# buggyyang/CDC_compression

Hardware: AMD Instinct MI355X
Metric: decoded images/sec at 256x256, 500-step x-param (higher is better)
Workload: dtype f32 (f16x2 split products)

## Files before the change

### cdc_compression_amd/csrc/cdc_internal.h

```cpp
#pragma once
#include <stdio.h>
#include <string.h>
#include <stdlib.h>
#include <hip/hip_runtime.h>
#include <map>
#include <mutex>
#include <utility>
#include <stdint.h>

#include <string>
#include <vector>

#include "conv_args.h"

extern "C" char **environ;

namespace cdc {

typedef void (*conv_kernel_fn)(const ConvArgs);
conv_kernel_fn conv_lookup_a(int MB, int NPW, int lnmode);
conv_kernel_fn conv_lookup_b(int MB, int NPW, int lnmode);
conv_kernel_fn conv_lookup_c(int MB, int NPW, int lnmode);
conv_kernel_fn conv_lookup_split(int MB, int NPW);
conv_kernel_fn conv_lookup_split2(int MB, int NPW, int lnmode, int xu = 1);
conv_kernel_fn conv_lookup_split2h(int MB, int NPW, int lnmode, int xu = 1);
conv_kernel_fn conv_lookup_split2hu(int MB, int NPW);

struct ConvShape {
    int Cin, Cout, KH, KW, stride;
    int C0 = 0;
    int Win = 0;
    int nz = 1, pad_x[4] = {0, 0, 0, 0};
    bool allow_split = false;
    int arith = 0;
    bool per_image_w = false;
    int Ho, Wo;
    int B;
    bool need_all_cout;
    int lnmode;
    int max_ksplit = 1;
};
bool conv_make_plan(const ConvShape &s, ConvPlan *plan);
hipError_t conv_launch(ConvArgs a, const ConvPlan &plan, int B, int nz, hipStream_t st);

struct PfShape {
    int Cin, Cout, C0 = 0, KH, KW, nz = 1, Ho, Wo, B;
    bool need_all_cout = false;
    int stride = 1;
    int uf = 0;
    int cop = 0;
    int tz = 1;
};
struct PfPlan {
    int MB, NPW, WM, WP, ring, tiles_x, tiles_y, groups; size_t lds_bytes; int lin = 0;
    int x16 = 0;
    int pf3_epv = 0, pf3_G = 0, pf3_iters = 0;
};
bool pf_make_plan(const PfShape &s, PfPlan *plan);
hipError_t pf_launch(PfArgs a, const PfPlan &plan, int B, int nz, hipStream_t st);
bool pf3_make_plan(const PfArgs &a, int B, int nz, PfPlan *plan);
hipError_t pf3_launch(PfArgs a, const PfPlan &plan, int B, hipStream_t st);
int device_cus();
struct WsPlan { int W, NPB, stride, waves, tiles, groups; size_t lds_bytes; };
struct WsArgs;
bool ws_make_plan(int Cin, int C0, int Cout, int H, int W, int B, int stride, WsPlan *plan);
hipError_t ws_launch(WsArgs a, const WsPlan &plan, hipStream_t st);
struct Ws1Plan { int NPB, waves, tiles, groups; size_t lds_bytes; };
struct Ws1Args;
bool ws1_make_plan(int Cin, int C0, int Cout, int HW, int B, bool per_image_w, Ws1Plan *plan);
hipError_t ws1_launch(Ws1Args a, const Ws1Plan &plan, hipStream_t st);
bool pw_make_plan(const PfShape &s, PfPlan *plan);
hipError_t pw_launch(PfArgs a, const PfPlan &plan, int B, hipStream_t st);
hipError_t pf_pack_launch(const float *src, long long src_bs, void *dst, long long dst_bs, int C, int H, int W, int B,
                          hipStream_t st);
hipError_t c4_pack_launch(const float *src, long long src_bs, float *dst, int C, long long HW, int B, hipStream_t st);
hipError_t pf_unpack_launch(const void *src, long long src_bs, float *dst, long long dst_bs, int C, int H, int W, int B, hipStream_t st);

inline const char *dev_env(const char *name) {
    static const bool on = [] {
        const char *e = ::getenv("CDC_DEV");
        if (e && atoi(e) != 0) return true;
        static const char *const user_level[] = {"CDC_DEV=", "CDC_ARITH=", "CDC_NO_RANGE_GUARD=", "CDC_GRAPH=", "CDC_DEBUG_PLAN=", "CDC_PROF_OPS=",
                                                 "CDC_BENCH_", "CDC_TEST_OBS=", "CDC_SYNC_EACH_OP=", "CDC_HIP_LIB=", "CDC_NO_COMBINE_FUSE="};
        for (char **v = environ; v && *v; ++v) {
            if (strncmp(*v, "CDC_", 4)) continue;
            bool user = false;
            for (const char *u : user_level) user = user || !strncmp(*v, u, strlen(u));
            if (!user) {
                fprintf(stderr, "cdc_hip: %.*s is set but ignored: development switches need CDC_DEV=1\n", (int)strcspn(*v, "="), *v);
                break;
            }
        }
        return false;
    }();
    return on ? ::getenv(name) : nullptr;
}

inline hipError_t ensure_dynamic_lds(const void *fn, size_t bytes) {
    if (bytes <= 64 * 1024) return hipSuccess;
    static std::mutex mu;
    static std::map<std::pair<int, const void *>, size_t> done;
    int dev = 0;
    (void)hipGetDevice(&dev);
    std::lock_guard<std::mutex> lk(mu);
    size_t &have = done[{dev, fn}];
    if (have >= bytes) return hipSuccess;
    hipError_t e = hipFuncSetAttribute(fn, hipFuncAttributeMaxDynamicSharedMemorySize, (int)bytes);
    if (e == hipSuccess) have = bytes;
// ... 181 lines not shown
```

### cdc_compression_amd/csrc/cdc_planner.hip

```cpp
#include "cdc_state.h"

namespace cdcapi {

constexpr int kKsTarget = 1024;

struct Builder {
    cdc_handle *h;
    int B;
    std::vector<void *> *pool;
    int rc = CDC_OK;
    int planB = 0;
    int pb() const { return planB > 0 ? planB : B; }
    std::vector<Op> *cur = nullptr;

    void emit(Op op) {
        op.id = (int)h->op_ms.size();
        h->op_ms.push_back(0); h->op_n.push_back(0); h->op_flops.push_back(op.flops);
        const bool hoisted = cur == &h->pre_ops;
        char buf[160];
        std::visit([&](const auto &payload) { op_label(payload, buf, sizeof buf, hoisted); }, op.p);
        if (hoisted && !strstr(buf, " HOIST") && strlen(buf) + 7 < sizeof buf) strcat(buf, " HOIST");
        h->op_label.push_back(buf);
        (cur ? cur : &h->ops)->push_back(op);
    }
// ... 275 lines not shown
                if (!tr->valid || tr->C != w.Cout || tr->H != Ho || tr->W != Wo || w.transposed || w.stride != 1 ||
                    o.resid_bs != (long long)w.Cout * Ho * Wo || o.resid_cs != (long long)Ho * Wo) {
                    if (!ensure_f32(o.resid, o.resid_bs)) {
                        if (!rc) rc = fail(h, CDC_ERR_UNSUPPORTED, "planes-only residual of a shape the plane-operand kernels do not read");
                        return true;
                    }
                } else {
                    a.resid = nullptr;
                    a.resid_pf = tr->p; a.rpf_bs = tr->bs(); a.rpf_ps = tr->ps(); a.rpf_ys = Wo + 2; a.rpf_zoff = (Wo + 2) + 1;
                }
            }
        if (planB == 0) pf3_make_plan(a, B, w.nz, &op.plan);
        if (debug_plan())
            fprintf(stderr, "[plan] conv %dx%d %d->%d out %dx%d on conv_pf%s_kernel (epv %d, %d workgroups x %d tiles per group)\n", w.KH, w.KW, w.Cin, w.Cout,
                    Ho, Wo, op.plan.pf3_epv ? "3" : "", op.plan.pf3_epv, op.plan.pf3_G, op.plan.pf3_iters);
        const double px = (double)B * Ho * Wo * w.nz;
        return finish(prof, op, 2.0 * px * w.Cout * w.Cin * w.KH * w.KW, 4.0 * ((double)B * w.Cin * H * W + px * w.Cout), a.out == nullptr);
    }

    bool try_pf_uf(const ConvW &w, const float *s0, long long bs0, int H, int W, float *out, long long out_bs, const ConvOpts &o,
                   bool need_all, int prof) {
        PfShape ps;
        if (!pf_on() || o.uf_c != 3 || o.uf_pad != 3 || !pf_uf_form(w, H, W, need_all, &ps)) return false;
        if (o.pre_mean || o.w_bs || o.wsp_bs || o.max_ksplit > 1 || o.resid || o.res3_w || o.stat_mean) return false;
        PfPlan plan;
        if (!pf_make_plan(ps, &plan)) return false;
        PfConvOp op;
        op.plan = plan; op.nz = 1;
        PfArgs &a = op.a;
        memset(&a, 0, sizeof a);
        a.x0 = s0; a.x0_bs = bs0;
        a.C0 = a.Cin = 32; a.H = H; a.W = W;
        a.w = w.wsh; a.w_zs = w.wsp_zs / 8;
        a.KH = 7; a.KW = 1; a.nz = 1;
        a.nchunk = 2; a.COP = w.COP; a.Cout = w.Cout;
        a.acc_scale = w.wscale_inv;
        out_geometry(a, w, H, W);
        a.out = out; a.out_bs = out_bs;
        if (o.emit_pf && bind_out_pf(a, w, out, out_bs, H, W) && o.no_f32) a.out = nullptr;
        const float *c4 = o.pre_add && cur != &h->pre_ops ? pre_add_c4(o.pre_add, w.Cout, H, W, out_bs) : nullptr;
        epilogue(a, w, o);
        if (c4) { a.pre_add = c4; a.pre_c4 = 1; }
        const double px = (double)B * H * W;
        return finish(prof, op, 2.0 * px * w.Cout * w.Cin * 7, 4.0 * ((double)B * 3 * H * W + px * w.Cout), a.out == nullptr);
    }

    bool try_pw(const ConvW &w, const float *s0, int C0, long long bs0, const float *s1, long long bs1, int H, int W,
                float *out, long long out_bs, const ConvOpts &o, bool need_all, int prof) {
        PfShape ps;
        if (h->arith != 1 || dev_env("CDC_NO_PW") || !pw_form(w, s1 ? C0 : 0, H, W, &ps)) return false;
        if (need_all || o.ln_g || o.stat_mean || o.res3_w || o.pf_only) return false;
        if (o.pre_mean && o.pre_mode != 2) return false;
        if (o.w_bs && !o.wsp_bs) return false;
        PfPlan plan;
        if (!pw_make_plan(ps, &plan)) return false;
        if (plan.lin && (o.shift || o.wsp_bs || (long long)w.Cout * H * W != out_bs)) return false;
        if (debug_plan())
            fprintf(stderr, "[plan] conv1x1 PW Cin=%4d Cout=%4d out=%3dx%-3d %s%s| MB=%d NPW=%d WM=%d WP=%d groups=%d R=%d wgs=%d lds=%zu\n", w.Cin, w.Cout,
                    H, W, o.pre_mean ? "pre2 " : "", o.wsp_bs ? "per-image " : "", plan.MB, plan.NPW, plan.WM, plan.WP, plan.groups, plan.ring,
                    plan.tiles_x * plan.tiles_y * B * plan.groups, plan.lds_bytes);
        PwConvOp op;
        op.plan = plan;
        PfArgs &a = op.a;
        memset(&a, 0, sizeof a);
        a.x0 = s0; a.x0_bs = bs0; a.x1 = s1; a.x1_bs = bs1;
        a.C0 = s1 ? C0 : w.Cin; a.Cin = w.Cin; a.H = H; a.W = W;
        a.pre_mean = o.pre_mean; a.pre_rstd = o.pre_mean ? o.pre_rstd : nullptr;
        a.w = w.wsh; a.w_bs = o.wsp_bs / 8;
        a.KH = 1; a.KW = 1; a.nz = 1;
        a.nchunk = w.Cin / 16; a.COP = w.COP; a.Cout = w.Cout;
        a.acc_scale = w.wscale_inv;
        out_geometry(a, w, H, W);
        a.out = out; a.out_bs = out_bs;
        if (o.emit_pf && !plan.lin && (w.Cout % 32) == 0 && bind_out_pf(a, w, out, out_bs, H, W) && o.no_f32) a.out = nullptr;
        epilogue(a, w, o);
        const double px = (double)B * H * W;
        return finish(prof, op, 2.0 * px * w.Cout * w.Cin, 4.0 * ((double)B * w.Cin * H * W + px * w.Cout), a.out == nullptr);
    }

    bool ws_would_plan(const ConvW &w, int C0, bool two_src, int H, int W, WsPlan *plan) {
        if (h->arith != 1 || !w.wsh || planB > 0 || w.KH != 3 || w.KW != 3 || (w.stride != 1 && w.stride != 2) || w.transposed || w.nz != 1) return false;
        if (w.py() != 1 || w.px() != 1) return false;
        if (w.COP != w.Cout || w.Cin_pad != w.Cin) return false;
        if (w.stride == 2 && ((H & 1) || (W & 1) || two_src)) return false;
        return ws_make_plan(w.Cin, two_src ? C0 : w.Cin, w.Cout, H / w.stride, W / w.stride, pb(), w.stride, plan);
    }
    bool try_ws(const ConvW &w, const float *s0, int C0, long long bs0, const float *s1, long long bs1, int H, int W, float *raw,
                long long raw_bs, int prof, const float *pre_add = nullptr) {
        WsConvOp op;
        if (rc || !ws_would_plan(w, C0, s1 != nullptr, H, W, &op.plan)) return false;
        if (!ensure_f32(s0, bs0) || (s1 && !ensure_f32(s1, bs1))) return false;
        const int Ho = H / w.stride, Wo = W / w.stride;
        if (raw_bs != (long long)w.Cout * Ho * Wo) return false;
        WsArgs &a = op.a;
        memset(&a, 0, sizeof a);
        a.x0 = s0; a.x0_bs = bs0; a.x1 = s1; a.x1_bs = bs1;
        a.C0 = s1 ? C0 : w.Cin; a.Cin = w.Cin; a.H = Ho; a.B = B;
        a.w = w.wsh; a.nchunk = w.Cin / 16; a.COP = w.COP; a.Cout = w.Cout; a.acc_scale = w.wscale_inv;
        a.bias = pre_add ? nullptr : w.bias;
        a.pre_add = pre_add;
        a.out = raw; a.out_bs = raw_bs;
        a.fault = fault_flag();
        if (debug_plan())
            fprintf(stderr, "[plan] conv 3x3 s%d %d->%d out %dx%d on conv_ws_kernel: %d tiles of %d pixels x %d groups, %d waves, %zu bytes of LDS\n", w.stride, w.Cin, w.Cout, Ho, Wo,
                    op.plan.tiles, op.plan.NPB * 32, op.plan.groups, op.plan.waves, op.plan.lds_bytes);
        const double px = (double)B * Ho * Wo;
        return finish(prof, op, 2.0 * px * w.Cout * w.Cin * 9, 4.0 * ((double)B * H * W * w.Cin + px * w.Cout), false);
    }

    bool try_ws1(const ConvW &w, const float *s0, int C0, long long bs0, const float *s1, long long bs1, int H, int W, float *out, long long out_bs,
                 const ConvOpts &o, bool need_all, int prof) {
        PfShape ps;
        if (rc || h->arith != 1 || planB > 0 || !pw_form(w, 0, H, W, &ps)) return false;
        if (need_all || o.ln_g || o.stat_mean || o.res3_w || o.pf_only || (o.pre_add && o.resid) || o.relu || o.resid1 || o.uf_c) return false;
        if (o.pre_mean && o.pre_mode != 2) return false;
        if (o.w_bs && !o.wsp_bs) return false;
        if (w.COP != w.Cout || w.Cin_pad != w.Cin || out_bs != (long long)w.Cout * H * W) return false;
        if (o.resid && (o.resid_cs != (long long)H * W)) return false;
        const long long blocks = (long long)pb() * (H * W / 32);
        const long long max_blocks = dev_env("CDC_WS1_MAX_BLOCKS") ? atoll(dev_env("CDC_WS1_MAX_BLOCKS")) : 128;
        const int max_groups_wide = dev_env("CDC_WS1_MAX_GROUPS") ? atoi(dev_env("CDC_WS1_MAX_GROUPS")) : 0;
        const bool wide_ok = blocks <= max_blocks || (max_groups_wide > 0 && blocks <= 256 && w.Cout / 32 <= max_groups_wide);
        if (!wide_ok && !(o.wsp_bs && W < 32)) return false;
        Ws1ConvOp op;
        op.H = H;
        if (!ws1_make_plan(w.Cin, s1 ? C0 : w.Cin, w.Cout, H * W, pb(), o.wsp_bs != 0, &op.plan)) return false;
        if (!ensure_f32(s0, bs0) || (s1 && !ensure_f32(s1, bs1)) || (o.resid && !ensure_f32(o.resid, o.resid_bs))) return false;
        Ws1Args &a = op.a;
// ... 1087 lines not shown
```

### cdc_compression_amd/csrc/cdc_state.h

```cpp
#pragma once
#include <math.h>
#include <stdarg.h>
#include <stdio.h>
#include <stdlib.h>
#include <string.h>

#include <algorithm>
#include <map>
#include <memory>
#include <string>
#include <variant>
#include <vector>

#include "../../include/cdc_hip.h"
#include "cdc_internal.h"
#include "conv_ws_kernel.h"
#include "conv_ws1_kernel.h"
#include "entropy.h"

using namespace cdc;

namespace cdcapi {


// ... 58 lines not shown
                               UnfoldArgs, VbrArgs, MaxpoolArgs, LpipsHeadArgs, GdnArgs>;

struct Op {
    int prof;
    int id = -1;
    double flops, bytes;
    OpPayload p;
    template <class T> Op(int prof_, const T &payload, double flops_ = 0, double bytes_ = 0) : prof(prof_), flops(flops_), bytes(bytes_), p(payload) {}
    template <class T> const T *get() const { return std::get_if<T>(&p); }
    bool on_conv_pf_kernel() const { return get<PfConvOp>() != nullptr; }
};

inline hipError_t op_launch(const ConvOp &o, int B, hipStream_t st) { return conv_launch(o.a, o.plan, B, o.nz, st); }
inline hipError_t op_launch(const PfConvOp &o, int B, hipStream_t st) { return pf_launch(o.a, o.plan, B, o.nz, st); }
inline hipError_t op_launch(const PwConvOp &o, int B, hipStream_t st) { return pw_launch(o.a, o.plan, B, st); }
inline hipError_t op_launch(const WsConvOp &o, int, hipStream_t st) { return ws_launch(o.a, o.plan, st); }
inline hipError_t op_launch(const Ws1ConvOp &o, int, hipStream_t st) { return ws1_launch(o.a, o.plan, st); }
inline hipError_t op_launch(const PfPackOp &o, int B, hipStream_t st) { return pf_pack_launch(o.src, o.src_bs, o.dst, o.dst_bs, o.C, o.H, o.W, B, st); }
inline hipError_t op_launch(const C4PackOp &o, int B, hipStream_t st) { return c4_pack_launch(o.src, o.src_bs, o.dst, o.C, (long long)o.H * o.W, B, st); }
inline hipError_t op_launch(const PfUnpackOp &o, int B, hipStream_t st) { return pf_unpack_launch(o.planes, o.planes_bs, o.dst, o.dst_bs, o.C, o.H, o.W, B, st); }
inline hipError_t op_launch(const LnArgs &a, int B, hipStream_t st) { return ln_launch(a, B, st); }
inline hipError_t op_launch(const TembArgs &a, int B, hipStream_t st) { return temb_launch(a, B, st); }
inline hipError_t op_launch(const KstatsOp &o, int B, hipStream_t st) { return kstats_launch(o.a, B, st); }
inline hipError_t op_launch(const CtxPartialOp &o, int B, hipStream_t st) { return ctx_partial_launch(o.a, B, st); }
inline hipError_t op_launch(const CtxOneOp &o, int B, hipStream_t st) { return ctx_one_launch(o.a, B, st); }
inline hipError_t op_launch(const CtxReduceOp &o, int B, hipStream_t st) { return ctx_reduce_launch(o.a, B, st); }
inline hipError_t op_launch(const CtxFoldOp &o, int B, hipStream_t st) { return ctx_fold_launch(o.a, B, st); }
inline hipError_t op_launch(const KvCtxArgs &a, int B, hipStream_t st) { return kvctx_launch(a, B, st); }
inline hipError_t op_launch(const LnConvArgs &a, int B, hipStream_t st) { return lnconv_launch(a, B, st); }
inline hipError_t op_launch(const CombineArgs &a, int B, hipStream_t st) { return fold_combine_launch(a, B, st); }
inline hipError_t op_launch(const DdimArgs &a, int, hipStream_t st) { return ddim_launch(a, st); }
inline hipError_t op_launch(const SolverArgs &a, int, hipStream_t st) { return solver_launch(a, st); }
inline hipError_t op_launch(const CopyArgs &a, int B, hipStream_t st) { return copy_channels_launch(a, B, st); }
inline hipError_t op_launch(const UnfoldArgs &a, int B, hipStream_t st) { return unfold_x_launch(a, B, st); }
inline hipError_t op_launch(const VbrArgs &a, int B, hipStream_t st) { return vbr_affine_launch(a, B, st); }
inline hipError_t op_launch(const MaxpoolArgs &a, int B, hipStream_t st) { return maxpool2_launch(a, B, st); }
inline hipError_t op_launch(const LpipsHeadArgs &a, int B, hipStream_t st) { return lpips_head_launch(a, B / 2, st); }
inline hipError_t op_launch(const GdnArgs &a, int B, hipStream_t st) { return gdn_launch(a, B, st); }

inline void op_label(const ConvOp &o, char *buf, size_t n, bool hoisted) {
    const ConvArgs &a = o.a; const ConvPlan &p = o.plan;
    snprintf(buf, n, "conv %dx%d s%d %4d->%-4d out %3dx%-3d MB%d NPW%d WN%d g%d tg%d ipw%d ks%d%s%s%s%s%s", a.KH, a.KW, a.stride, a.Cin, a.Cout, a.Ho,
             a.Wo, p.MB, p.NPW, p.WN, p.groups, p.tg, p.ipw, p.ksplit, p.split == 2 ? (p.arith ? " SPLIT2H" : " SPLIT2") : (p.split ? " SPLIT" : ""),
             a.ep_g ? " LN" : "", a.ln_mean ? " pre" : "", hoisted ? " HOIST" : "", a.resid ? " +res" : "");
}
inline void pf_label(const PfArgs &a, const PfPlan &p, const char *kernel, char *buf, size_t n, bool hoisted) {
    snprintf(buf, n, "conv %dx%d s%d %4d->%-4d out %3dx%-3d MB%d NPW%d WM%d WP%d g%d R%d %s%s%s%s%s%s", a.KH, a.KW, a.stride == 2 ? 2 : 1, a.Cin, a.Cout,
             a.Ho, a.Wo, p.MB, p.NPW, p.WM, p.WP, p.groups, p.ring, kernel, a.out ? "" : " nof32", a.out_pf ? " +pf" : "",
             a.resid ? " +res" : (a.resid_pf ? " +resP" : ""), hoisted ? " HOIST" : "", a.tz == 4 ? " TZ4" : "");
}
inline void op_label(const PfConvOp &o, char *buf, size_t n, bool hoisted) {
    pf_label(o.a, o.plan, o.plan.pf3_epv ? (o.a.ep_g ? "PF3 LN" : "PF3") : (o.a.ep_g ? "PF LN" : "PF"), buf, n, hoisted);
}
inline void op_label(const PwConvOp &o, char *buf, size_t n, bool hoisted) { pf_label(o.a, o.plan, o.a.pre_mean ? "PW pre" : "PW", buf, n, hoisted); }
inline void op_label(const WsConvOp &o, char *buf, size_t n, bool) {
    snprintf(buf, n, "conv 3x3 s%d %4d->%-4d out %3dx%-3d NPB%d waves%d tiles%d g%d WS%s", o.plan.stride, o.a.Cin, o.a.Cout, o.a.H, o.plan.W, o.plan.NPB,
             o.plan.waves, o.plan.tiles, o.plan.groups, o.a.pre_add ? " pre_add" : "");
}
inline void op_label(const Ws1ConvOp &o, char *buf, size_t n, bool) {
    snprintf(buf, n, "conv 1x1 s1 %4d->%-4d out %3dx%-3d NPB%d waves%d tiles%d g%d WS1%s%s%s", o.a.Cin, o.a.Cout, o.H, o.a.HW / std::max(o.H, 1), o.plan.NPB,
             o.plan.waves, o.plan.tiles, o.plan.groups, o.a.pre_mean ? " pre" : "", o.a.w_bs ? " perimg" : "",
             o.a.resid ? (o.a.resid_is_pre ? " pre_add" : " +res") : "");
}
inline void op_label(const PfPackOp &, char *buf, size_t n, bool) { snprintf(buf, n, "pfpack"); }
inline void op_label(const C4PackOp &, char *buf, size_t n, bool) { snprintf(buf, n, "pfpack"); }
inline void op_label(const PfUnpackOp &, char *buf, size_t n, bool) { snprintf(buf, n, "pfunpack"); }
inline void op_label(const LnArgs &a, char *buf, size_t n, bool) { snprintf(buf, n, "ln C=%d HW=%d%s", a.C, a.HW, a.out ? "" : " stats"); }
inline void op_label(const TembArgs &, char *buf, size_t n, bool) { snprintf(buf, n, "temb"); }
inline void ctx_label(const char *kind, const AttnCtxArgs &a, int nsplit, char *buf, size_t n) { snprintf(buf, n, "%s C=%d N=%d nsplit=%d", kind, a.C, a.N, nsplit); }
inline void op_label(const KstatsOp &o, char *buf, size_t n, bool) { ctx_label("kstats", o.a, o.a.nsplit, buf, n); }
inline void op_label(const CtxPartialOp &o, char *buf, size_t n, bool) { ctx_label("ctxp", o.a, o.a.nsplit, buf, n); }
inline void op_label(const CtxOneOp &o, char *buf, size_t n, bool) { ctx_label("ctx1", o.a, 1, buf, n); }
inline void op_label(const CtxReduceOp &o, char *buf, size_t n, bool) { ctx_label("ctxr", o.a, o.a.nsplit, buf, n); }
inline void op_label(const CtxFoldOp &o, char *buf, size_t n, bool) { ctx_label("ctxf", o.a, o.a.nsplit, buf, n); }
inline void op_label(const KvCtxArgs &a, char *buf, size_t n, bool) { snprintf(buf, n, "kvctx C=%d N=%d nsplit=%d", a.C, a.N, a.nsplit); }
inline void op_label(const LnConvArgs &a, char *buf, size_t n, bool) { snprintf(buf, n, "lnconv C=%d N=%d nsplit=%d", a.C, a.N, a.nsplit); }
inline void op_label(const CombineArgs &, char *buf, size_t n, bool) { snprintf(buf, n, "combine"); }
inline void op_label(const DdimArgs &, char *buf, size_t n, bool) { snprintf(buf, n, "ddim"); }
inline void op_label(const SolverArgs &, char *buf, size_t n, bool) { snprintf(buf, n, "solver"); }
inline void op_label(const CopyArgs &, char *buf, size_t n, bool) { snprintf(buf, n, "copy"); }
inline void op_label(const UnfoldArgs &, char *buf, size_t n, bool) { snprintf(buf, n, "unfold"); }
inline void op_label(const VbrArgs &a, char *buf, size_t n, bool) { snprintf(buf, n, "vbr C=%d HW=%d%s", a.C, a.HW, a.leaky ? " leaky" : ""); }
inline void op_label(const MaxpoolArgs &a, char *buf, size_t n, bool) { snprintf(buf, n, "maxpool2 C=%d in %dx%d", a.C, a.H, a.W); }
inline void op_label(const LpipsHeadArgs &a, char *buf, size_t n, bool) { snprintf(buf, n, "lpips_head tap %d C=%d HW=%d", a.layer, a.C, a.HW); }
inline void op_label(const GdnArgs &a, char *buf, size_t n, bool) { snprintf(buf, n, "gdn C=%d HW=%d%s", a.C, a.HW, a.inverse ? " inv" : ""); }

struct GdnW { int C = 0; bool inverse = false; float *beta = nullptr, *gamma = nullptr; };
struct VbrW { int C = 0; float *p = nullptr; };


}
using namespace cdcapi;

static int default_arith() {
    const char *e = getenv("CDC_ARITH");
    return e ? (atoi(e) ? 1 : 0) : 1;
}

template <class T> struct GrowBuf {
    T *p = nullptr;
    size_t cap = 0;
    int grow(cdc_handle *h, size_t n);
    void release() { if (p) (void)hipFree(p); p = nullptr; cap = 0; }
};
template <class T> struct StagedBuf {
    GrowBuf<T> dev;
    std::vector<T> host;
// ... 272 lines not shown
```

### cdc_compression_amd/csrc/conv_args.h

```cpp
#pragma once
#include <stdint.h>

namespace cdc {

constexpr int kWaveSize = 64;
constexpr int kXS = 20;

struct ConvArgs {
    const float *src0, *src1;
    long long src0_bs, src1_bs;
    int uf_c, uf_pad;
    unsigned uf_magic;
    int C0, Cin;
    int H, W;
    const float *ln_mean, *ln_rstd;
    const float *ln_g, *ln_b;
    const float *wp;
    long long w_bs, w_zs;
    const unsigned short *wsp;
    long long wsp_zs;
    long long wsp_bs;
    float acc_scale;
    int tg;
    int ipw, B;
// ... 33 lines not shown
    int *fault;
#ifdef CDC_TIMELINE
    unsigned long long *tl;
#endif
};

struct PfArgs {
    const void *src0, *src1;
    long long src0_bs, src1_bs;
    int C0, Cin;
    int H, W;
    const void *w;
    long long w_zs;
    int KH, KW, nz;
    int stride;
    int tz;
    int pad_y[4], pad_x[4];
    int nchunk, COP, Cout;
    float acc_scale;
    int ring;
    int n_iter;
    float *out;
    long long out_bs, out_cs;
    int out_ys, out_xs, out_zoff[4];
    void *out_pf;
    long long pf_bs, pf_ps;
    int pf_ys, pf_xs, pf_zoff[4];
    int Ho, Wo;
    int lognbw, tiles_x, tiles_y, B;
    int xcd_remap;
    const float *bias, *pre_add, *ep_g, *ep_b;
    int pre_c4;
    float eps;
    int relu;
    float relu_slope;
    const float *shift;
    int shift_bs;
    const float *resid;
    long long resid_bs, resid_cs;
    const float *resid1;
    long long resid1_bs;
    int resid_c0;
    const void *resid_pf;
    long long rpf_bs, rpf_ps;
    int rpf_ys, rpf_zoff;
    float *stat_mean, *stat_rstd;
    const float *res3_w, *res3_x;
    long long res3_bs;
    const float *x0, *x1;
    long long x0_bs, x1_bs;
    const float *pre_mean, *pre_rstd;
    long long w_bs;
    int lin;
    int dbg;
    int *fault;
#ifdef CDC_TIMELINE
    unsigned long long *tl;
#endif
};

constexpr int kPfXS = 12;

struct ConvPlan {
    int MB, NPW, WN;
    int groups;
    int KC, nchunk;
    int lognbw, tiles_x, tiles_y, PH, PW;
    int xvec, xshift[4];
    size_t lds_bytes;
    int lnmode;
    int tg;
    int ipw;
    int ksplit = 1;
    int xu = 1;
    int arith = 0;
    int split;
};

}
```

### cdc_compression_amd/csrc/conv_inst_w.hip

```cpp
#include <algorithm>
#include <map>
#include <string>
#include <vector>
#include <stdlib.h>

#include "cdc_internal.h"
#include "conv_pw_kernel.h"

namespace cdc {

typedef void (*pw_kernel_fn)(const PfArgs);
static pw_kernel_fn pw_lookup(int MB, int NPW, int WM, int WP, bool x16 = false) {
    if (x16) {
        if (MB == 2 && NPW == 2 && WM == 1 && WP == 4) return conv_pw_kernel<2, 2, 1, 4, true>;
        if (MB == 2 && NPW == 2 && WM == 2 && WP == 2) return conv_pw_kernel<2, 2, 2, 2, true>;
        if (MB == 2 && NPW == 2 && WM == 4 && WP == 2) return conv_pw_kernel<2, 2, 4, 2, true>;
        if (MB == 3 && NPW == 1 && WM == 2 && WP == 4) return conv_pw_kernel<3, 1, 2, 4, true>;
        return nullptr;
    }
    if (MB == 2 && NPW == 2 && WM == 1 && WP == 4) return conv_pw_kernel<2, 2, 1, 4>;
    if (MB == 2 && NPW == 2 && WM == 2 && WP == 2) return conv_pw_kernel<2, 2, 2, 2>;
    if (MB == 2 && NPW == 2 && WM == 4 && WP == 2) return conv_pw_kernel<2, 2, 4, 2>;
    if (MB == 3 && NPW == 1 && WM == 2 && WP == 4) return conv_pw_kernel<3, 1, 2, 4>;
    return nullptr;
}
struct PwCand { int MB, NPW, WM, WP; };
static const PwCand kPwCands[] = {
    {2, 2, 4, 2},
    {3, 1, 2, 4},
    {2, 2, 2, 2},
    {2, 2, 1, 4},
};

bool pw_make_plan(const PfShape &s, PfPlan *p) {
    if (s.KH != 1 || s.KW != 1 || s.nz != 1) return false;
    if (s.Cout % 32 || s.Cin % 16 || (s.C0 % 16) || s.Cin < 32) return false;
    const bool lin = s.Wo < 32;
    if (lin && ((s.Ho * s.Wo) % 32)) return false;
    const double min_waves = dev_env("CDC_PW_MIN_WAVES") ? atof(dev_env("CDC_PW_MIN_WAVES")) : 512.0;
    const bool x16 = (lin || ((s.Wo & 3) == 0 && s.Wo >= 4)) && !dev_env("CDC_NO_PW_X16");
    double best = -1;
    for (const PwCand &c : kPwCands) {
        const int COPT = c.WM * c.MB * 32, NW = c.WM * c.WP;
        if (s.Cout % COPT) continue;
        if (s.need_all_cout && COPT != s.Cout) continue;
        const int ring = pw_ring(c.MB, c.NPW, c.WM, c.WP, x16);
        if (ring < 5 || s.Cin / 16 < 2) continue;
        const int TH = c.WP * c.NPW;
        const int groups = s.Cout / COPT;
        const long long nb = (long long)s.B * (s.Ho * s.Wo / 32);
        const double wgs = lin ? (double)((nb + TH - 1) / TH) * groups
                               : (double)((s.Wo + 31) / 32) * ((s.Ho + TH - 1) / TH) * s.B * groups;
        if (wgs * NW < min_waves) continue;
        const double fill = std::min(1.0, wgs * NW / 2048.0);
        const double score = fill / (1.0 + 0.25 * (groups - 1)) * (c.MB * c.NPW >= 4 ? 1.0 : 0.8);
        if (score > best) {
            best = score;
            p->MB = c.MB; p->NPW = c.NPW; p->WM = c.WM; p->WP = c.WP;
            p->ring = ring;
            p->lin = lin ? 1 : 0;
            p->tiles_x = lin ? (int)((nb + TH - 1) / TH) : (s.Wo + 31) / 32;
            p->tiles_y = lin ? 1 : (s.Ho + TH - 1) / TH;
            p->groups = groups;
            p->lds_bytes = (size_t)ring * pf_rows(c.MB, c.NPW) * COPT * 16 + pw_x_bytes(c.NPW, c.WM, c.WP, x16);
            p->x16 = x16 ? 1 : 0;
        }
    }
    return best >= 0;
}

hipError_t pw_launch(PfArgs a, const PfPlan &p, int B, hipStream_t st) {
    pw_kernel_fn fn = pw_lookup(p.MB, p.NPW, p.WM, p.WP, p.x16 != 0);
    if (!fn) return hipErrorInvalidValue;
    a.lognbw = 5;
    a.tiles_x = p.tiles_x; a.tiles_y = p.tiles_y; a.B = B; a.ring = p.ring;
    if (hipError_t e = ensure_dynamic_lds((const void *)fn, p.lds_bytes); e != hipSuccess) return e;
    a.lin = p.lin;
    if (const char *e = dev_env("CDC_PW_DBG")) a.dbg = atoi(e); else
    a.dbg = dev_env("CDC_PW_COUNTED_WAIT") ? 1024 : 0;
    dim3 grid((unsigned)(p.lin ? p.tiles_x : p.tiles_x * p.tiles_y * B), (unsigned)p.groups, 1);
    a.xcd_remap = (grid.x % 8 == 0 && grid.x >= 64) ? 1 : 0;
#ifdef CDC_TIMELINE
    static unsigned long long *tl_dev = nullptr;
    static std::map<std::string, int> seen;
    const size_t tl_wgs = (size_t)grid.x * grid.y;
    char key[96];
    snprintf(key, sizeof key, "pw 1x1 %d->%d out %dx%d", a.Cin, a.Cout, a.Ho, a.Wo);
    a.tl = nullptr;
    if (tl_wgs <= (1u << 18) && seen[key]++ < 2) {
        if (!tl_dev) hipMalloc(&tl_dev, sizeof(unsigned long long) * 16 * (1u << 18));
        hipMemsetAsync(tl_dev, 0, sizeof(unsigned long long) * 16 * tl_wgs, st);
        a.tl = tl_dev;
    }
#endif
    hipLaunchKernelGGL(fn, grid, dim3(64 * p.WM * p.WP), p.lds_bytes, st, a);
#ifdef CDC_TIMELINE
    if (a.tl) {
        hipStreamSynchronize(st);
        std::vector<unsigned long long> h(16 * tl_wgs);
        hipMemcpy(h.data(), tl_dev, h.size() * 8, hipMemcpyDeviceToHost);
        double cat[7] = {0}, life = 0;
        for (size_t w = 0; w < tl_wgs; ++w) {
            const unsigned long long *r = &h[w * 16];
            for (int c = 0; c < 7; ++c) cat[c] += (double)r[c];
            life += (double)(r[8] - r[7]);
        }
        static const char *names[7] = {"setup", "prologue issue", "prologue wait", "main loop", "epilogue parameters", "-", "epilogue blocks"};
        fprintf(stderr, "[pf timeline] conv %s: %zu workgroups x %d threads, lds %zu; mean workgroup life %.0f; per workgroup (wave 0):", key, tl_wgs, 64 * p.WM * p.WP, p.lds_bytes,
                life / tl_wgs);
        for (int c = 0; c < 7; ++c) fprintf(stderr, "  %s %.0f", names[c], cat[c] / tl_wgs);
        fprintf(stderr, "\n");
    }
#endif
    return hipGetLastError();
}

}
```

### cdc_compression_amd/csrc/conv_pw_kernel.h

```cpp
#pragma once
#include "conv_pf_kernel.h"

namespace cdc {

constexpr int kPwPD = 2;
constexpr int kPwX16N = 2 * 256 + 32;
__host__ __device__ constexpr size_t pw_x_bytes(int NPW, int WM, int WP, bool X16 = false) {
    return (size_t)WM * WP * kPwPD * NPW * (X16 ? kPwX16N * 4 : 8 * 256);
}
__host__ __device__ constexpr int pw_ring(int MB, int NPW, int WM, int WP, bool X16 = false) {
    const size_t budget = (WM * WP == 8 ? 150 * 1024 : 78 * 1024) - pw_x_bytes(NPW, WM, WP, X16);
    const size_t wst = (size_t)pf_rows(MB, NPW) * WM * MB * 32 * 16;
    const int r = (int)(budget / wst);
    return r > 6 ? 6 : r;
}

__device__ __forceinline__ void dma4(unsigned voff, const void *sbase, unsigned lds_byte) {
    asm volatile("s_mov_b32 m0, %2\n\ts_nop 0\n\tglobal_load_lds_dword %0, %1" ::"v"(voff), "s"(sbase), "s"(lds_byte)
                 : "memory");
}

template <int MB, int NPW, int WM, int WP, bool X16 = false>
__global__ void __launch_bounds__(64 * WM * WP, WM * WP == 8 ? 1 : 2) conv_pw_kernel(const PfArgs P) {
    constexpr int NW = WM * WP, NT = 64 * NW, COPT = WM * MB * 32;
    static_assert(COPT % 64 == 0, "a weight DMA instruction (64 units) must stay inside one (plane, k-half) row");
    constexpr bool ACC2 = pf_acc2(MB, NPW);
    constexpr int NPL = ACC2 ? 2 : 3, ROWS = 2 * NPL;
    constexpr int WI = ROWS * COPT / 64;
    constexpr int NWW = (WI + NW - 1) / NW;
    constexpr int WST = ROWS * COPT;
    constexpr int R = pw_ring(MB, NPW, WM, WP, X16);
    static_assert(R >= 5, "no room for the weight ring");
    constexpr int TH = WP * NPW;
    constexpr int PD = kPwPD;
    extern __shared__ __attribute__((aligned(16))) uint4 smem_u[];
#ifdef CDC_TIMELINE
    unsigned long long tl_acc[7] = {0, 0, 0, 0, 0, 0, 0}, tl_last = __builtin_readcyclecounter();
    const unsigned long long tl_start = tl_last;
#endif
    const int tid = threadIdx.x, lane = tid & 63;
    const int wave = __builtin_amdgcn_readfirstlane(tid >> 6);
    const int wm = wave / WP, wp = wave % WP;
    const int cog = blockIdx.y;
    unsigned bid0 = blockIdx.x;
    if (P.xcd_remap) bid0 = (bid0 & 7) * (gridDim.x >> 3) + (bid0 >> 3);
    int bid = (int)bid0;
    const int tile = bid;
    const int tx = bid % P.tiles_x;
    bid /= P.tiles_x;
    const int ty = bid % P.tiles_y;
    const int b = P.lin ? 0 : bid / P.tiles_y;
    const int oy0 = ty * TH, ox0 = tx * 32;
    const int S = P.nchunk;
    const unsigned lds0 = __builtin_amdgcn_readfirstlane((unsigned)(size_t)(const __attribute__((address_space(3))) uint4 *)smem_u);

    const char *wsrc = reinterpret_cast<const char *>(P.w) + ((size_t)b * P.w_bs + (size_t)cog * COPT) * 16;
    unsigned wvo[NWW], wdo[NWW];
#pragma unroll
    for (int k = 0; k < NWW; ++k) {
        const int jj = min(wave + k * NW, WI - 1);
        const int row = jj / (COPT / 64), seg = jj - row * (COPT / 64);
        wvo[k] = (unsigned)(row * P.COP + seg * 64 + lane) * 16u;
        wdo[k] = __builtin_amdgcn_readfirstlane((unsigned)jj * 1024u);
    }
    const long long w_dc = (long long)6 * P.COP * 16;
    const char *wptr = wsrc;
    int sw = 0;
    auto issue_w = [&]() {
        const unsigned dst = lds0 + (unsigned)(sw * WST) * 16u;
#pragma unroll
        for (int k = 0; k < NWW; ++k) dma16(wvo[k], wptr, dst + wdo[k]);
        wptr += w_dc;
        if (++sw == R) sw = 0;
    };

    const int half = lane >> 5, j = lane & 31;
    const int HW = P.H * P.W;
    unsigned xvo[NPW];
    float mu[NPW];
    bool valid[NPW];
    unsigned pixo[NPW];
    int bimg[NPW];
    const int bpi = HW >> 5;
#pragma unroll
    for (int n = 0; n < NPW; ++n) {
        if (P.lin) {
            const int gb = tile * TH + wp * NPW + n, nb = P.B * bpi;
            valid[n] = gb < nb;
            const int gc = min(gb, nb - 1);
            bimg[n] = __builtin_amdgcn_readfirstlane(gc / bpi);
            pixo[n] = (unsigned)((gc - bimg[n] * bpi) * 32 + j);
        } else {
            const int oy = oy0 + wp * NPW + n, ox = ox0 + j;
            valid[n] = oy < P.Ho && ox < P.Wo;
            bimg[n] = b;
            pixo[n] = (unsigned)(min(oy, P.Ho - 1) * P.W + min(ox, P.Wo - 1));
        }
        xvo[n] = ((unsigned)(8 * half) * (unsigned)HW + pixo[n]) * 4u;
        if constexpr (X16) {
            const int r = lane >> 3, q = lane & 7;
            unsigned p4;
            if (P.lin) p4 = pixo[n] - (unsigned)j + 4u * q;
            else {
                const int oy = oy0 + wp * NPW + n;
                p4 = (unsigned)(min(oy, P.Ho - 1) * P.W + min(ox0 + 4 * q, P.Wo - 4));
            }
// ... 82 lines not shown
    };

    PFTL(0);
#pragma unroll
    for (int d = 0; d < PD; ++d)
        if (d < S) issue_x(d, d);
    for (int q = 0; q < R - 1 && q < S; ++q) issue_w();
    PFTL(1);
    dma_wait();
    __builtin_amdgcn_s_barrier();
    PFTL(2);
    OpsA A0, A1;
    OpsB B0, B1;
    fetch_a(a_base, A0);
    split_b(0, B0);
    if (PD < S) issue_x(PD, 0);
    int sn = 0;
    auto step = [&](int s, auto slotc, OpsA &Ac, OpsB &Bc, OpsA &An, OpsB &Bn) {
        constexpr int slot = decltype(slotc)::value;
        if (s + 1 < S) {
            if (++sn == R) sn = 0;
            if (s >= PD && s + R - 1 < S && s + 1 + PD < S && (P.dbg & 1024)) {
                if (P.dbg & 2048) vm_wait<(PD - 1) * (L + NWW)>(); else vm_wait<NWW + (PD - 1) * (L + NWW)>();
                if (P.dbg & 4096) __builtin_amdgcn_s_sleep(4);
            } else dma_wait();
            __builtin_amdgcn_s_barrier();
            fetch_a(a_base + sn * WST, An);
            split_b(slot, Bn);
#ifdef CDC_PW_LATE_PROBE
            if (P.dbg & 8192) {
                if (P.dbg & 16384) __builtin_amdgcn_s_sleep(16);
                OpsB Bt;
                split_b(slot, Bt);
                unsigned late = 0;
#pragma unroll
                for (int n = 0; n < NPW; ++n) {
                    bool d = false;
#pragma unroll
                    for (int i = 0; i < 8; ++i) d |= (float)Bn[0][n][i] != (float)Bt[0][n][i] || (float)Bn[1][n][i] != (float)Bt[1][n][i];
                    if (__any(d)) late |= 1u << n;
                }
                if (late && lane == 0)
                    printf("[pw late piece] workgroup (%d,%d) wave %d step %d of %d: pixel-block mask %x differs between the read behind vmcnt(%d) and a second read\n",
                           (int)blockIdx.x, (int)blockIdx.y, wave, s + 1, S, late, NWW + (PD - 1) * (L + NWW));
            }
#endif
            if (s + 1 + PD < S) issue_x(s + 1 + PD, slot);
            if (s + R - 1 < S) issue_w();
        }
        __builtin_amdgcn_s_setprio(2);
        mma(Ac, Bc);
        __builtin_amdgcn_s_setprio(0);
    };
    static_assert(PD == 2 && R >= PD + 3, "two activation stages; W(s+1) must be older than the activation pieces of step s+1");
    using P0 = std::integral_constant<int, 0>;
    using P1 = std::integral_constant<int, 1>;
    {
        int s = 0;
        for (; s + 1 < S; s += 2) {
            step(s, P1{}, A0, B0, A1, B1);
            step(s + 1, P0{}, A1, B1, A0, B0);
        }
        if (s < S) step(s, P1{}, A0, B0, A1, B1);
    }

    __builtin_amdgcn_s_barrier();
    PFTL(3);
    float *ep = reinterpret_cast<float *>(smem_u);
    for (int i = tid; i < COPT; i += NT) {
        const int co = cog * COPT + i;
        const bool ok = co < P.Cout;
        ep[i] = (ok && P.bias) ? P.bias[co] : 0.f;
        ep[COPT + i] = (ok && P.shift) ? P.shift[(size_t)b * P.shift_bs + co] : 0.f;
    }
    __syncthreads();
    PFTL(4);
    const int cobase = cog * COPT + wm * MB * 32;
    const float *epl = ep + wm * MB * 32 + 4 * half;
    const bool ch_ok = cobase + MB * 32 <= P.Cout;
#pragma unroll
    for (int n = 0; n < NPW; ++n) {
        const int oy = oy0 + wp * NPW + n, ox = ox0 + j;
        const int bn = bimg[n];
        const bool ok = valid[n] && ch_ok;
        const float sc = P.pre_rstd ? P.acc_scale * P.pre_rstd[(size_t)bn * HW + pixo[n]] : P.acc_scale;
        const size_t opix = P.lin ? (size_t)pixo[n] : (size_t)oy * P.out_ys + (size_t)ox * P.out_xs + P.out_zoff[0];
#pragma unroll
        for (int m = 0; m < MB; ++m)
#pragma unroll
            for (int r = 0; r < 16; ++r)
                acc[m][n][r] = (ACC2 ? acc[m][n][r] + acc2[ACC2 ? m : 0][ACC2 ? n : 0][r] * (1.0f / 2048.0f) : acc[m][n][r]) * sc +
                               epl[m * 32 + (r & 3) + 8 * (r >> 2)];
        if (!ok) continue;
        if (P.fault) {
            float s = 0.f;
#pragma unroll
            for (int m = 0; m < MB; ++m)
#pragma unroll
                for (int r = 0; r < 16; ++r) s += fabsf(acc[m][n][r]);
            if (!(s < 3.0e38f)) *P.fault = 1;
        }
        if (P.pre_add) {
            const float *pp = P.pre_add + (size_t)bn * P.out_bs + opix + (size_t)(cobase + 4 * half) * P.out_cs;
#pragma unroll
            for (int m = 0; m < MB; ++m)
#pragma unroll
                for (int r = 0; r < 16; ++r) acc[m][n][r] += pp[(size_t)(m * 32 + (r & 3) + 8 * (r >> 2)) * P.out_cs];
        }
        if (P.relu) {
#pragma unroll
            for (int m = 0; m < MB; ++m)
#pragma unroll
                for (int r = 0; r < 16; ++r) acc[m][n][r] = fmaxf(acc[m][n][r], P.relu_slope * acc[m][n][r]);
        }
        if (P.shift) {
#pragma unroll
            for (int m = 0; m < MB; ++m)
#pragma unroll
                for (int r = 0; r < 16; ++r) acc[m][n][r] += epl[COPT + m * 32 + (r & 3) + 8 * (r >> 2)];
        }
        if (P.resid) {
            const float *rp = P.resid + (size_t)bn * P.resid_bs + opix + (size_t)(cobase + 4 * half) * P.resid_cs;
#pragma unroll
            for (int m = 0; m < MB; ++m)
#pragma unroll
                for (int r = 0; r < 16; ++r) acc[m][n][r] += rp[(size_t)(m * 32 + (r & 3) + 8 * (r >> 2)) * P.resid_cs];
        }
        if (P.out) {
            float *op = P.out + (size_t)bn * P.out_bs + opix + (size_t)(cobase + 4 * half) * P.out_cs;
#pragma unroll
            for (int m = 0; m < MB; ++m)
#pragma unroll
                for (int r = 0; r < 16; ++r) op[(size_t)(m * 32 + (r & 3) + 8 * (r >> 2)) * P.out_cs] = acc[m][n][r];
        }
        if (P.out_pf) {
            const long long u0 = (long long)bn * P.pf_bs + (long long)oy * P.pf_ys + (long long)ox * P.pf_xs + P.pf_zoff[0];
#pragma unroll
            for (int m = 0; m < MB; ++m)
                pf_store_block(reinterpret_cast<uint4 *>(P.out_pf), u0 + (long long)((cobase >> 3) + m * 4) * 2 * P.pf_ps, P.pf_ps, half, acc[m][n]);
        }
    }
    PFTL(6);
    PFTL_END();
}

}
```

Measured before the change: 5.425.

## Keep full input tile resident in LDS for 1x1 conv residual reuse

Adds a specialized pointwise-conv kernel variant for the 64->64 channel case where the residual is the conv's own input. The whole activation tile (all 4 chunks) is staged in LDS instead of a 2-deep ring, so the residual add in the epilogue reads the input from LDS rather than reloading it from global memory. This saves one full-tensor global read per such layer, at the cost of more LDS per workgroup, a smaller MB/NPW configuration and possibly lower occupancy.

Measured after the change: 5.443, median of 6. No clear change (+0.3%).

```diff
diff --git a/cdc_compression_amd/csrc/cdc_internal.h b/cdc_compression_amd/csrc/cdc_internal.h
--- a/cdc_compression_amd/csrc/cdc_internal.h
+++ b/cdc_compression_amd/csrc/cdc_internal.h
@@ -50,10 +50,12 @@
     int uf = 0;
     int cop = 0;
     int tz = 1;
+    bool resx = false;
 };
 struct PfPlan {
     int MB, NPW, WM, WP, ring, tiles_x, tiles_y, groups; size_t lds_bytes; int lin = 0;
     int x16 = 0;
+    int resx = 0;
     int pf3_epv = 0, pf3_G = 0, pf3_iters = 0;
 };
 bool pf_make_plan(const PfShape &s, PfPlan *plan);
diff --git a/cdc_compression_amd/csrc/cdc_planner.hip b/cdc_compression_amd/csrc/cdc_planner.hip
--- a/cdc_compression_amd/csrc/cdc_planner.hip
+++ b/cdc_compression_amd/csrc/cdc_planner.hip
@@ -351,6 +351,7 @@
         if (need_all || o.ln_g || o.stat_mean || o.res3_w || o.pf_only) return false;
         if (o.pre_mean && o.pre_mode != 2) return false;
         if (o.w_bs && !o.wsp_bs) return false;
+        ps.resx = o.resid && o.resid == s0 && !s1 && !o.resid1 && o.resid_bs == bs0 && o.resid_cs == (long long)H * W && w.Cout == w.Cin;
         PfPlan plan;
         if (!pw_make_plan(ps, &plan)) return false;
         if (plan.lin && (o.shift || o.wsp_bs || (long long)w.Cout * H * W != out_bs)) return false;
@@ -373,6 +374,7 @@
         a.out = out; a.out_bs = out_bs;
         if (o.emit_pf && !plan.lin && (w.Cout % 32) == 0 && bind_out_pf(a, w, out, out_bs, H, W) && o.no_f32) a.out = nullptr;
         epilogue(a, w, o);
+        a.resx = plan.resx;
         const double px = (double)B * H * W;
         return finish(prof, op, 2.0 * px * w.Cout * w.Cin, 4.0 * ((double)B * w.Cin * H * W + px * w.Cout), a.out == nullptr);
     }
diff --git a/cdc_compression_amd/csrc/cdc_state.h b/cdc_compression_amd/csrc/cdc_state.h
--- a/cdc_compression_amd/csrc/cdc_state.h
+++ b/cdc_compression_amd/csrc/cdc_state.h
@@ -134,7 +134,10 @@
 inline void op_label(const PfConvOp &o, char *buf, size_t n, bool hoisted) {
     pf_label(o.a, o.plan, o.plan.pf3_epv ? (o.a.ep_g ? "PF3 LN" : "PF3") : (o.a.ep_g ? "PF LN" : "PF"), buf, n, hoisted);
 }
-inline void op_label(const PwConvOp &o, char *buf, size_t n, bool hoisted) { pf_label(o.a, o.plan, o.a.pre_mean ? "PW pre" : "PW", buf, n, hoisted); }
+inline void op_label(const PwConvOp &o, char *buf, size_t n, bool hoisted) {
+    pf_label(o.a, o.plan, o.a.pre_mean ? "PW pre" : "PW", buf, n, hoisted);
+    if (o.a.resx) snprintf(buf + strlen(buf), n - strlen(buf), " resx");
+}
 inline void op_label(const WsConvOp &o, char *buf, size_t n, bool) {
     snprintf(buf, n, "conv 3x3 s%d %4d->%-4d out %3dx%-3d NPB%d waves%d tiles%d g%d WS%s", o.plan.stride, o.a.Cin, o.a.Cout, o.a.H, o.plan.W, o.plan.NPB,
              o.plan.waves, o.plan.tiles, o.plan.groups, o.a.pre_add ? " pre_add" : "");
diff --git a/cdc_compression_amd/csrc/conv_args.h b/cdc_compression_amd/csrc/conv_args.h
--- a/cdc_compression_amd/csrc/conv_args.h
+++ b/cdc_compression_amd/csrc/conv_args.h
@@ -109,6 +109,7 @@
     const float *pre_mean, *pre_rstd;
     long long w_bs;
     int lin;
+    int resx;
     int dbg;
     int *fault;
 #ifdef CDC_TIMELINE
diff --git a/cdc_compression_amd/csrc/conv_inst_w.hip b/cdc_compression_amd/csrc/conv_inst_w.hip
--- a/cdc_compression_amd/csrc/conv_inst_w.hip
+++ b/cdc_compression_amd/csrc/conv_inst_w.hip
@@ -10,7 +10,11 @@
 namespace cdc {
 
 typedef void (*pw_kernel_fn)(const PfArgs);
-static pw_kernel_fn pw_lookup(int MB, int NPW, int WM, int WP, bool x16 = false) {
+static pw_kernel_fn pw_lookup(int MB, int NPW, int WM, int WP, bool x16 = false, int resx = 0) {
+    if (resx) {
+        if (x16 && resx == 4 && MB == 2 && NPW == 1 && WM == 1 && WP == 4) return conv_pw_kernel<2, 1, 1, 4, true, 4>;
+        return nullptr;
+    }
     if (x16) {
         if (MB == 2 && NPW == 2 && WM == 1 && WP == 4) return conv_pw_kernel<2, 2, 1, 4, true>;
         if (MB == 2 && NPW == 2 && WM == 2 && WP == 2) return conv_pw_kernel<2, 2, 2, 2, true>;
@@ -31,6 +35,20 @@
     {2, 2, 2, 2},
     {2, 2, 1, 4},
 };
+
+static bool pw_resx_plan(const PfShape &s, bool lin, bool x16, PfPlan *p) {
+    if (!s.resx || lin || !x16 || dev_env("CDC_NO_PW_RESX")) return false;
+    const PwCand c = {2, 1, 1, 4};
+    const int COPT = c.WM * c.MB * 32, RES = s.Cin / 16, TH = c.WP * c.NPW;
+    if (s.Cin != s.Cout || s.C0 || s.Cout != COPT || RES != 4 || !pw_lookup(c.MB, c.NPW, c.WM, c.WP, true, RES)) return false;
+    const int ring = pw_ring(c.MB, c.NPW, c.WM, c.WP, true, RES);
+    if (ring != RES) return false;
+    p->MB = c.MB; p->NPW = c.NPW; p->WM = c.WM; p->WP = c.WP;
+    p->ring = ring; p->lin = 0; p->x16 = 1; p->resx = RES;
+    p->tiles_x = (s.Wo + 31) / 32; p->tiles_y = (s.Ho + TH - 1) / TH; p->groups = 1;
+    p->lds_bytes = (size_t)ring * pf_rows(c.MB, c.NPW) * COPT * 16 + pw_x_bytes(c.NPW, c.WM, c.WP, true, RES);
+    return true;
+}
 
 bool pw_make_plan(const PfShape &s, PfPlan *p) {
     if (s.KH != 1 || s.KW != 1 || s.nz != 1) return false;
@@ -66,12 +84,13 @@
             p->x16 = x16 ? 1 : 0;
         }
     }
+    if (best >= 0) pw_resx_plan(s, lin, x16, p);
     return best >= 0;
 }
 
 hipError_t pw_launch(PfArgs a, const PfPlan &p, int B, hipStream_t st) {
-    pw_kernel_fn fn = pw_lookup(p.MB, p.NPW, p.WM, p.WP, p.x16 != 0);
-    if (!fn) return hipErrorInvalidValue;
+    pw_kernel_fn fn = pw_lookup(p.MB, p.NPW, p.WM, p.WP, p.x16 != 0, p.resx);
+    if (!fn || (p.resx && (a.resx != p.resx || a.nchunk != p.resx))) return hipErrorInvalidValue;
     a.lognbw = 5;
     a.tiles_x = p.tiles_x; a.tiles_y = p.tiles_y; a.B = B; a.ring = p.ring;
     if (hipError_t e = ensure_dynamic_lds((const void *)fn, p.lds_bytes); e != hipSuccess) return e;
diff --git a/cdc_compression_amd/csrc/conv_pw_kernel.h b/cdc_compression_amd/csrc/conv_pw_kernel.h
--- a/cdc_compression_amd/csrc/conv_pw_kernel.h
+++ b/cdc_compression_amd/csrc/conv_pw_kernel.h
@@ -5,13 +5,15 @@
 
 constexpr int kPwPD = 2;
 constexpr int kPwX16N = 2 * 256 + 32;
-__host__ __device__ constexpr size_t pw_x_bytes(int NPW, int WM, int WP, bool X16 = false) {
-    return (size_t)WM * WP * kPwPD * NPW * (X16 ? kPwX16N * 4 : 8 * 256);
-}
-__host__ __device__ constexpr int pw_ring(int MB, int NPW, int WM, int WP, bool X16 = false) {
-    const size_t budget = (WM * WP == 8 ? 150 * 1024 : 78 * 1024) - pw_x_bytes(NPW, WM, WP, X16);
+__host__ __device__ constexpr size_t pw_x_bytes(int NPW, int WM, int WP, bool X16 = false, int RES = 0) {
+    return (size_t)WM * WP * (RES ? RES : kPwPD) * NPW * (X16 ? kPwX16N * 4 : 8 * 256);
+}
+__host__ __device__ constexpr int pw_ring(int MB, int NPW, int WM, int WP, bool X16 = false, int RES = 0) {
+    const size_t total = WM * WP == 8 ? 150 * 1024 : 78 * 1024, xb = pw_x_bytes(NPW, WM, WP, X16, RES);
+    if (xb >= total) return 0;
     const size_t wst = (size_t)pf_rows(MB, NPW) * WM * MB * 32 * 16;
-    const int r = (int)(budget / wst);
+    const int r = (int)((total - xb) / wst);
+    if (RES) return r >= RES ? RES : 0;
     return r > 6 ? 6 : r;
 }
 
@@ -20,7 +22,7 @@
                  : "memory");
 }
 
-template <int MB, int NPW, int WM, int WP, bool X16 = false>
+template <int MB, int NPW, int WM, int WP, bool X16 = false, int RES = 0>
 __global__ void __launch_bounds__(64 * WM * WP, WM * WP == 8 ? 1 : 2) conv_pw_kernel(const PfArgs P) {
     constexpr int NW = WM * WP, NT = 64 * NW, COPT = WM * MB * 32;
     static_assert(COPT % 64 == 0, "a weight DMA instruction (64 units) must stay inside one (plane, k-half) row");
@@ -29,10 +31,10 @@
     constexpr int WI = ROWS * COPT / 64;
     constexpr int NWW = (WI + NW - 1) / NW;
     constexpr int WST = ROWS * COPT;
-    constexpr int R = pw_ring(MB, NPW, WM, WP, X16);
-    static_assert(R >= 5, "no room for the weight ring");
+    constexpr int R = pw_ring(MB, NPW, WM, WP, X16, RES);
+    static_assert(RES ? (R == RES && X16 && RES == 4) : R >= 5, "no room for the weight ring");
     constexpr int TH = WP * NPW;
-    constexpr int PD = kPwPD;
+    constexpr int PD = RES ? RES : kPwPD;
     extern __shared__ __attribute__((aligned(16))) uint4 smem_u[];
 #ifdef CDC_TIMELINE
     unsigned long long tl_acc[7] = {0, 0, 0, 0, 0, 0, 0}, tl_last = __builtin_readcyclecounter();
@@ -51,7 +53,7 @@
     const int ty = bid % P.tiles_y;
     const int b = P.lin ? 0 : bid / P.tiles_y;
     const int oy0 = ty * TH, ox0 = tx * 32;
-    const int S = P.nchunk;
+    const int S = RES ? RES : P.nchunk;
     const unsigned lds0 = __builtin_amdgcn_readfirstlane((unsigned)(size_t)(const __attribute__((address_space(3))) uint4 *)smem_u);
 
     const char *wsrc = reinterpret_cast<const char *>(P.w) + ((size_t)b * P.w_bs + (size_t)cog * COPT) * 16;
@@ -240,10 +242,15 @@
         mma(Ac, Bc);
         __builtin_amdgcn_s_setprio(0);
     };
-    static_assert(PD == 2 && R >= PD + 3, "two activation stages; W(s+1) must be older than the activation pieces of step s+1");
+    static_assert(RES || (PD == 2 && R >= PD + 3), "two activation stages; W(s+1) must be older than the activation pieces of step s+1");
     using P0 = std::integral_constant<int, 0>;
     using P1 = std::integral_constant<int, 1>;
-    {
+    if constexpr (RES) {
+        step(0, P1{}, A0, B0, A1, B1);
+        step(1, std::integral_constant<int, 2>{}, A1, B1, A0, B0);
+        step(2, std::integral_constant<int, 3>{}, A0, B0, A1, B1);
+        step(3, P0{}, A1, B1, A0, B0);
+    } else {
         int s = 0;
         for (; s + 1 < S; s += 2) {
             step(s, P1{}, A0, B0, A1, B1);
@@ -307,7 +314,16 @@
 #pragma unroll
                 for (int r = 0; r < 16; ++r) acc[m][n][r] += epl[COPT + m * 32 + (r & 3) + 8 * (r >> 2)];
         }
-        if (P.resid) {
+        if constexpr (RES) {
+            const float *rp = xw + ((cobase >> 4) * XST + n * kPwX16N + half * (4 * 32) + j);
+#pragma unroll
+            for (int m = 0; m < MB; ++m)
+#pragma unroll
+                for (int r = 0; r < 16; ++r) {
+                    const int c = m * 32 + 8 * (r >> 2);
+                    acc[m][n][r] += rp[(c >> 4) * XST + ((c >> 3) & 1) * (256 + 32) + (r & 3) * 32];
+                }
+        } else if (P.resid) {
             const float *rp = P.resid + (size_t)bn * P.resid_bs + opix + (size_t)(cobase + 4 * half) * P.resid_cs;
 #pragma unroll
             for (int m = 0; m < MB; ++m)
```
